# kuanyuke/BayHunter

Hardware: AMD Instinct MI355X
Metric: forward evals/sec (SWD+RF, 10-layer) (higher is better)
Workload: dtype f64; 1 GPU; joint10: rdispph+prf(201 samples, nsamp 512), 10 layers, 21 periods, 524288 models/GPU/step; models_per_gpu=524288, err_models=0, library=bayhunter_amd 0.2 (gfx950) src 067974131c026079, overlap=True

## Files before the change

### bayhunter_amd/csrc/kernels.hip

```cpp
#include <hip/hip_runtime.h>
#include <cstdlib>
#include "kernels.h"
#include "rf_core.h"
#include "swd_core.h"
#include "swd_team.h"

namespace bh {

static hipError_t ensure_dyn_lds(const void *func, size_t lds, size_t (&set)[16])
{
    if (lds <= 48 * 1024) return hipSuccess;
    int dev = 0;
    hipError_t e = hipGetDevice(&dev);
    if (e != hipSuccess) return e;
    dev &= 15;
    if (lds > set[dev]) {
        e = hipFuncSetAttribute(func, hipFuncAttributeMaxDynamicSharedMemorySize, (int)lds);
        if (e != hipSuccess) return e;
        set[dev] = lds;
    }
    return hipSuccess;
}

struct LdsLay {
    float *base;
    int L;
    __device__ __forceinline__ float d(int i) const { return base[(0 * L + i) * SWD_T]; }
    __device__ __forceinline__ float a(int i) const { return base[(1 * L + i) * SWD_T]; }
    __device__ __forceinline__ float b(int i) const { return base[(2 * L + i) * SWD_T]; }
    __device__ __forceinline__ float rho(int i) const { return base[(3 * L + i) * SWD_T]; }
    __device__ __forceinline__ void set_d(int i, float v) { base[(0 * L + i) * SWD_T] = v; }
    __device__ __forceinline__ void set_a(int i, float v) { base[(1 * L + i) * SWD_T] = v; }
    __device__ __forceinline__ void set_b(int i, float v) { base[(2 * L + i) * SWD_T] = v; }
    __device__ __forceinline__ void set_rho(int i, float v) { base[(3 * L + i) * SWD_T] = v; }
};

__device__ __forceinline__ void swd_bad_depth(const SwdArgs &A, const SwdTargetDev &tg, int t, long b)
{
    double *out = A.out + b * A.out_stride + tg.out_off;
    for (int k = 0; k < tg.nper; k++) out[k] = __builtin_nan("");
    A.err[b * A.ntargets + t] = 2;
}

struct QueueSrc {
    const SwdArgs &A;
    const SwdTargetDev &tg;
    unsigned int *counter;
    int t;
    long cur;
    __device__ __forceinline__ int next(LdsLay &lay, double *&out, double *&cws, double *&cbws)
    {
        unsigned int b;
        int nl;
        const int L = A.Lmax;
        for (;;) {
            b = atomicAdd(counter, 1u);
            if (b >= (unsigned int)A.B) return 0;
            if (A.order) b = (unsigned int)A.order[b];
            nl = A.nlay[b];
            if (nl >= 1 && nl <= L) break;
            swd_bad_depth(A, tg, t, b);
        }
        cur = b;
        const long g = (long)b * A.mstride;
        if (A.vec2) {
            constexpr int CH = 6;
            for (int l0 = 0; l0 < nl; l0 += 2 * CH) {
                double2 p[CH], q[CH];
#pragma unroll
                for (int u = 0; u < CH; u++)
                    if (l0 + 2 * u < nl) {
                        p[u] = *(const double2 *)(A.h + g + l0 + 2 * u);
                        q[u] = *(const double2 *)(A.vp + g + l0 + 2 * u);
                    }
#pragma unroll
                for (int u = 0; u < CH; u++) {
                    const int l = l0 + 2 * u;
                    if (l < nl) { lay.set_d(l, (float)p[u].x); lay.set_a(l, (float)q[u].x); }
                    if (l + 1 < nl) { lay.set_d(l + 1, (float)p[u].y); lay.set_a(l + 1, (float)q[u].y); }
                }
#pragma unroll
                for (int u = 0; u < CH; u++)
                    if (l0 + 2 * u < nl) {
                        p[u] = *(const double2 *)(A.vs + g + l0 + 2 * u);
                        q[u] = *(const double2 *)(A.rho + g + l0 + 2 * u);
                    }
#pragma unroll
                for (int u = 0; u < CH; u++) {
                    const int l = l0 + 2 * u;
                    if (l < nl) { lay.set_b(l, (float)p[u].x); lay.set_rho(l, (float)q[u].x); }
                    if (l + 1 < nl) { lay.set_b(l + 1, (float)p[u].y); lay.set_rho(l + 1, (float)q[u].y); }
                }
            }
        } else {
            for (int l = 0; l < nl; l++) {
                lay.set_d(l, (float)A.h[g + l]);
                lay.set_a(l, (float)A.vp[g + l]);
                lay.set_b(l, (float)A.vs[g + l]);
                lay.set_rho(l, (float)A.rho[g + l]);
            }
        }
        out = A.out + (long)b * A.out_stride + tg.out_off;
        if (tg.mode > 1) {
            cws = A.ws + ((long)t * 2 * BH_NP) * A.B + b;
            cbws = cws + (long)BH_NP * A.B;
        }
        return nl;
    }
    float *stage;
    __device__ __forceinline__ void put(SwdState &S, int k, int kmax, float v)
    {
        if (stage) stage[(k - 1) * SWD_T] = v;
        else swd_put_direct(S, k, kmax, v);
    }
    __device__ __forceinline__ void fill_zero(SwdState &S, int k, int kmax)
    {
        if (stage) { for (int i = k; i <= kmax; i++) stage[(i - 1) * SWD_T] = 0.f; }
        else swd_zero_direct(S, k, kmax);
    }
    __device__ __forceinline__ void done(int err)
    {
        A.err[cur * A.ntargets + t] = err;
        if (stage) {
            const int n = tg.nper;
            double *o = A.out + cur * A.out_stride + tg.out_off;
            int k = 0;
            if (((unsigned long long)o & 15) && n > 0) { o[0] = (double)stage[0]; k = 1; }
            for (; k + 1 < n; k += 2) swd_store_pair(o + k, stage[k * SWD_T], stage[(k + 1) * SWD_T]);
            if (k < n) o[k] = (double)stage[k * SWD_T];
        }
    }
    __device__ __forceinline__ void sphere(LdsLay &lay, int mmax, int ifunc) { swd_sphere(lay, mmax, ifunc); }
};

#ifndef BH_SWD_WAVES
#define BH_SWD_WAVES 2
#endif
#if defined(BH_LANE_PROFILE)
__device__ unsigned long long g_lane_prof[8];
template <class Lay, class Src>
__device__ __forceinline__ void swd_lane_prof(Lay &lay, Src &src, const SwdTargetDev &tg, const double *BH_RESTRICT per, int wss)
{
    SwdState S;
    swd_state_init(S);
    NevRegs nv;
    swd_nev_init(nv);
    nv.cycles = 0;
    unsigned long long td = 0, te = 0, tc = 0, n = 0, t0 = clock64(), t1;
    for (;;) {
        swd_events(S, lay, src, tg, per, wss);
        t1 = clock64(); td += t1 - t0; t0 = t1;
        if (S.st == SWD_ST_DONE) break;
        const double wvno = S.omega / S.ceval;
        const double del = (tg.iwave == 1) ? swd_dltar1(lay, S.mmax, S.llw, wvno, S.omega)
                                           : swd_dltar4(lay, S.mmax, S.llw, wvno, S.omega);
        t1 = clock64(); te += t1 - t0; t0 = t1;
        swd_control(S, del, nv);
        t1 = clock64(); tc += t1 - t0; t0 = t1;
        n++;
    }
    atomicAdd(&g_lane_prof[0], td);
    atomicAdd(&g_lane_prof[1], te);
    atomicAdd(&g_lane_prof[2], tc);
    atomicAdd(&g_lane_prof[3], n);
    atomicAdd(&g_lane_prof[4], nv.cycles);
}
extern "C" int bh_debug_lane_profile(unsigned long long *out, int reset)
{
    if (out && hipMemcpyFromSymbol(out, HIP_SYMBOL(g_lane_prof), sizeof(g_lane_prof)) != hipSuccess) return 1;
    if (reset) {
        unsigned long long z[8] = {0};
        if (hipMemcpyToSymbol(HIP_SYMBOL(g_lane_prof), z, sizeof(z)) != hipSuccess) return 1;
    }
    return 0;
}
#endif
__global__ __launch_bounds__(SWD_T) __attribute__((amdgpu_waves_per_eu(BH_SWD_WAVES, BH_SWD_WAVES))) void swd_kernel(SwdArgs A)
{
    extern __shared__ float lds[];
    const int t = blockIdx.y;
    if (!((A.tmask >> t) & 1u)) return;
    const SwdTargetDev tg = A.tg[t];
    LdsLay lay{lds + threadIdx.x, A.Lmax};
    QueueSrc src{A, tg, A.counters + t, t, 0, A.stage ? lds + 4 * A.Lmax * SWD_T + threadIdx.x : nullptr};
    double *perl = (double *)(lds + (4 * A.Lmax + A.stage) * SWD_T);
    for (int k = threadIdx.x; k < tg.nper; k += SWD_T) perl[k] = A.periods[tg.per_off + k];
    __syncthreads();
#if defined(BH_LANE_PROFILE)
    swd_lane_prof(lay, src, tg, perl, A.B);
#else
    swd_lane(lay, src, tg, perl, A.B, nullptr);
#endif
}

struct TeamLay {
    float *base;
    int L;
    __device__ __forceinline__ float d(int i) const { return base[i]; }
    __device__ __forceinline__ float a(int i) const { return base[L + i]; }
    __device__ __forceinline__ float b(int i) const { return base[2 * L + i]; }
    __device__ __forceinline__ float rho(int i) const { return base[3 * L + i]; }
    __device__ __forceinline__ void set_d(int i, float v) { base[i] = v; }
    __device__ __forceinline__ void set_a(int i, float v) { base[L + i] = v; }
    __device__ __forceinline__ void set_b(int i, float v) { base[2 * L + i] = v; }
    __device__ __forceinline__ void set_rho(int i, float v) { base[3 * L + i] = v; }
};

struct TeamSrc {
    const SwdArgs &A;
    const SwdTargetDev &tg;
    int t, lane, nlanes, taken;
    long b;
    unsigned int *queue;
    float *res;
    __device__ __forceinline__ int next(TeamLay &lay, double *&out, double *&cws, double *&cbws)
    {
        const int L = A.Lmax;
        int nl;
        for (;;) {
            if (queue) {
                int nb = 0;
                if (lane == 0) nb = (int)atomicAdd(queue, 1u);
                nb = __shfl(nb, (int)(threadIdx.x & 63) - lane, 64);
                if (nb >= A.B) return 0;
                b = A.order ? A.order[nb] : nb;
            } else {
                if (taken) return 0;
                taken = 1;
                if (A.order) b = A.order[b];
            }
            nl = A.nlay[b];
            if (nl >= 1 && nl <= L) break;
            if (lane == 0) swd_bad_depth(A, tg, t, b);
        }
        const long g = b * A.mstride;
        for (int l = lane; l < nl; l += nlanes) {
            lay.set_d(l, (float)A.h[g + l]);
            lay.set_a(l, (float)A.vp[g + l]);
            lay.set_b(l, (float)A.vs[g + l]);
            lay.set_rho(l, (float)A.rho[g + l]);
        }
        __syncthreads();
        out = A.out + b * A.out_stride + tg.out_off;
        if (tg.mode > 1) {
            cws = A.ws + ((long)t * 2 * BH_NP) * A.B + b;
            cbws = cws + (long)BH_NP * A.B;
        }
        return nl;
    }
    __device__ __forceinline__ void done(int err)
    {
        if (lane == 0) A.err[b * A.ntargets + t] = err;
        if (res && lane < tg.nper)
            A.out[b * A.out_stride + tg.out_off + lane] = (double)res[lane];
    }
    __device__ __forceinline__ void put(SwdState &S, int k, int kmax, float v)
    {
        if (res) { if (lane == 0) res[k - 1] = v; return; }
        if (lane == 0) swd_put_direct(S, k, kmax, v);
        else if ((k & 1) && k != kmax) S.pend = v;
    }
    __device__ __forceinline__ void fill_zero(SwdState &S, int k, int kmax)
    {
        if (res) {
            if (lane == 0)
                for (int i = k; i <= kmax; i++) res[i - 1] = 0.f;
            return;
        }
        if (lane == 0) swd_zero_direct(S, k, kmax);
    }
    __device__ __forceinline__ void sphere(TeamLay &lay, int mmax, int ifunc)
    {
        if (threadIdx.x < SWD_T) swd_sphere(lay, mmax, ifunc);
        __syncthreads();
    }
};

#if defined(BH_TEAM_PROFILE)
__device__ unsigned long long g_team_prof[20];
#define BH_TP_DECL unsigned long long tp_[18] = {0, 0, 0, 0, 0, 0, 0, 0, 0, 0, 0, 0, 0, 0, 0, 0, 0, 0}, tp_t0_ = clock64(), tp_t1_
#define BH_TP(i) (tp_t1_ = clock64(), tp_[i] += tp_t1_ - tp_t0_, tp_t0_ = tp_t1_)
#define BH_TP_COUNT(i, n) (tp_[i] += (n))
#define BH_TP_FLUSH(rounds)                                                                  \
    if (threadIdx.x == 0) {                                                                  \
        for (int i_ = 0; i_ < 18; i_++) atomicAdd(&g_team_prof[i_], tp_[i_]);                \
        atomicAdd(&g_team_prof[18], (unsigned long long)(rounds));                           \
        atomicAdd(&g_team_prof[19], 1ull);                                                   \
    }
#else
#define BH_TP_DECL
#define BH_TP(i)
#define BH_TP_COUNT(i, n)
#define BH_TP_FLUSH(rounds)
#endif

template <int TEAM>
__device__ __forceinline__ void swd_team_body(const SwdArgs &A)
{
    extern __shared__ double tlds[];
    constexpr int NSUB = SWD_T / TEAM;
    static_assert(NSUB > 1, "64 lanes and more per search: swd_teamw_body");
    const int sub = threadIdx.x / TEAM, lane = threadIdx.x % TEAM;
    const int t = blockIdx.y;
    if (!((A.tmask >> t) & 1u)) return;
    const SwdTargetDev tg = A.tg[t];
    const int nm = A.Lmax > TEAM ? A.Lmax : TEAM;
    const int per_team = nm * SWD_NCA + 2 * SWD_TEAM_NT + (4 * A.Lmax + 1) / 2;
    double *mats = tlds + (long)sub * per_team, *trials = mats + (long)nm * SWD_NCA, *dels = trials + SWD_TEAM_NT;
    TeamLay lay{(float *)(dels + SWD_TEAM_NT), A.Lmax};
    TeamSrc src{A, tg, t, lane, TEAM, 0, (long)blockIdx.x, A.counters + t, nullptr};
    const double *per = A.periods + tg.per_off;
    SwdState S;
    swd_state_init(S);
    NevRegs nv;
    swd_nev_init(nv);
    {
        bool live = true;
        for (;;) {
            if (live) {
                swd_events(S, lay, src, tg, per, A.B);
                live = S.st != SWD_ST_DONE;
            }
            if (!__any(live)) break;
            const int nt = live ? swd_team_plan(S, TEAM, trials) : 0;
            __syncthreads();
            swd_team_assemble(lay, lane, TEAM, tg.iwave, S, nt, trials, mats);
            __syncthreads();
            if (tg.iwave == 2 && 8 * nt <= TEAM) swd_team_chain_ray5(lay, lane, S, nt, trials, mats, dels);
            else swd_team_chain(lay, lane, tg.iwave, S, nt, trials, mats, dels);
            __syncthreads();
            swd_team_consume(S, nv, nt, trials, dels);
            __syncthreads();
        }
    }
}


template <int CTRL>
__device__ __forceinline__ double dpp_quad(double x)
{
    const int lo = __builtin_amdgcn_mov_dpp(__double2loint(x), CTRL, 0xF, 0xF, true);
    const int hi = __builtin_amdgcn_mov_dpp(__double2hiint(x), CTRL, 0xF, 0xF, true);
    return __hiloint2double(hi, lo);
}
__device__ __forceinline__ double readlane_d(double x, int j)
{
    const int lo = __builtin_amdgcn_readlane(__double2loint(x), j);
    const int hi = __builtin_amdgcn_readlane(__double2hiint(x), j);
    return __hiloint2double(hi, lo);
}

__device__ __forceinline__ double uni(double x)
{
    return __hiloint2double(__builtin_amdgcn_readfirstlane(__double2hiint(x)),
                            __builtin_amdgcn_readfirstlane(__double2loint(x)));
}
__device__ __forceinline__ int uni(int x) { return __builtin_amdgcn_readfirstlane(x); }
__device__ __forceinline__ float uni(float x) { return __int_as_float(__builtin_amdgcn_readfirstlane(__float_as_int(x))); }
template <class T>
__device__ __forceinline__ T *uni(T *p)
{
    const unsigned long long v = (unsigned long long)p;
    return (T *)(((unsigned long long)(unsigned)__builtin_amdgcn_readfirstlane((int)(v >> 32)) << 32) |
                 (unsigned)__builtin_amdgcn_readfirstlane((int)v));
}
struct LdsSlots {
    const double *d, *tc;
    __device__ __forceinline__ double del(int j) const { return d[j]; }
    __device__ __forceinline__ double c(int j) const { return tc[j]; }
};
struct TeamwVals {
    double mc, mom, dl;
    int nt;
    TeamwNode nd;
    unsigned long long left, right;
#if defined(BH_TEAM_PROFILE)
    unsigned long long *tp, *t0;
    __device__ __forceinline__ void probe(int i) const { const unsigned long long t = clock64(); tp[i] += t - *t0; *t0 = t; }
    __device__ __forceinline__ void count(int i, int n) const { tp[i] += n; }
#else
    __device__ __forceinline__ void probe(int) const {}
    __device__ __forceinline__ void count(int, int) const {}
#endif
    __device__ __forceinline__ int find(double om, double c) const
    {
        const unsigned long long m = __ballot(mc == c && mom == om && (int)(threadIdx.x & 63) < nt);
        return m ? __ffsll((long long)m) - 1 : -1;
    }
    __device__ __forceinline__ double del(int j) const { return readlane_d(dl, j); }
    __device__ __forceinline__ double c(int j) const { return readlane_d(mc, j); }
    __device__ __forceinline__ int go(const SwdState &, int j) const
    {
        return ((right >> j) & 1) ? SWD_GO_RIGHT : ((left >> j) & 1) ? SWD_GO_LEFT : SWD_GO_STOP;
    }
    __device__ __forceinline__ int chain_run(const SwdState &, int first, int dir, int max) const
    {
        const unsigned long long m = (dir == SWD_GO_RIGHT ? right : left) >> first;
        const unsigned long long stop = ~m & 0x5555555555555555ull;
        const int n = stop ? (__ffsll((long long)stop) - 1) >> 1 : 32;
        return n < max ? n : max;
    }
    __device__ __forceinline__ TeamwNode node(const SwdState &, int j) const
    {
        TeamwNode a;
        a.go = SWD_GO_STOP;
        a.out = __builtin_amdgcn_readlane(nd.out, j);
        a.c1 = readlane_d(nd.c1, j); a.d1 = readlane_d(nd.d1, j);
        a.c2 = readlane_d(nd.c2, j); a.d2 = readlane_d(nd.d2, j);
        a.c3n = readlane_d(nd.c3n, j);
        return a;
    }
    __device__ __forceinline__ int run(int first, int stride, int count, bool neg) const
    {
        const bool same = (mc == mc) && ((__double2hiint(dl) < 0) == neg) && (int)(threadIdx.x & 63) < nt;
        unsigned long long m = __ballot(same) >> first;
        int n;
        if (stride == 2) {
            const unsigned long long stop = ~m & 0x5555555555555555ull;
            n = stop ? (__ffsll((long long)stop) - 1) >> 1 : 32;
        } else {
            const unsigned long long stop = ~m;
            n = stop ? __ffsll((long long)stop) - 1 : 64;
        }
        return n < count ? n : count;
    }
};

template <int K>
struct SubVals {
    double mc, mom, dl;
    int nt, tl, base;
    const double *tc, *dls, *ndc;
    const int *nout;
    unsigned long long left, right;
    static constexpr unsigned long long MASK = (1ull << K) - 1;
    __device__ __forceinline__ void probe(int) const {}
    __device__ __forceinline__ void count(int, int) const {}
    __device__ __forceinline__ unsigned long long mine(bool p) const { return (__ballot(p) >> base) & MASK; }
    __device__ __forceinline__ int find(double om, double c) const
    {
        const unsigned long long m = mine(mc == c && mom == om && tl < nt);
        return m ? __ffsll((long long)m) - 1 : -1;
    }
    __device__ __forceinline__ double del(int j) const { return dls[j]; }
    __device__ __forceinline__ double c(int j) const { return tc[j]; }
    __device__ __forceinline__ int go(const SwdState &, int j) const
    {
        return ((right >> j) & 1) ? SWD_GO_RIGHT : ((left >> j) & 1) ? SWD_GO_LEFT : SWD_GO_STOP;
    }
    __device__ __forceinline__ int chain_run(const SwdState &, int first, int dir, int max) const
    {
        const unsigned long long m = (dir == SWD_GO_RIGHT ? right : left) >> first;
        const unsigned long long stop = ~m & 0x5555555555555555ull;
        const int n = stop ? (__ffsll((long long)stop) - 1) >> 1 : 32;
// ... 622 lines not shown
```

### bayhunter_amd/csrc/swd_core.h

```cpp
#pragma once
#include "bh_common.h"
#include "bh_math.h"

namespace bh {

struct VarProd {
    double a0, cpcq, cpy, cpz, cqw, cqx, xy, xz, wy, wz;
};

BH_DEV void swd_var(double p, double q, const Recip &by_ra, const Recip &by_rb, double wvno, double xka,
                    double xkb, double dpth, double *w_out, double *cosp_out, VarProd &o)
{
    const double ra = by_ra.b, rb = by_rb.b;
    double w, x, y, z, cosp, cosq, sinp, sinq, fac;
    double pex = 0.0, sex = 0.0;
    if (wvno < xka) {
        bh_sincos(p, &sinp, &cosp);
        w = qdiv(sinp, by_ra);
        x = -ra * sinp;
    } else if (wvno == xka) {
        cosp = 1.0; w = dpth; x = 0.0;
    } else {
        pex = p;
        fac = 0.0;
// ... 43 lines not shown
    const Recip by_rho = recip_of(rho);
    a.c12 = qdiv(wvno2 * v.cpy - v.cqx, by_rho);
    a.c13 = qdiv(-(twgm1 * a0pq + gammk * v.xz + wvno2 * gamm1 * v.wy), by_rho);
    a.c14 = qdiv(v.cpz - wvno2 * v.cqw, by_rho);
    a.c15 = qdiv(-(two * wvno2 * a0pq + v.xz + wvno2 * wvno2 * v.wy), recip_sq(by_rho));
    a.c21 = (gmgmk * v.cpz - gm1sq * v.cqw) * rho;
    a.c22 = v.cpcq;
    a.c23 = gammk * v.cpz - gamm1 * v.cqw;
    a.c24 = -v.wz;
    a.c41 = (gm1sq * v.cpy - gmgmk * v.cqx) * rho;
    a.c42 = -v.xy;
    a.c43 = gamm1 * v.cpy - gammk * v.cqx;
    a.c51 = -(two * gmgmk * gm1sq * a0pq + gmgmk * gmgmk * v.xz + gm1sq * gm1sq * v.wy) * rho2;
    a.c53 = -(gammk * gamm1 * twgm1 * a0pq + gam * gammk * gammk * v.xz + gamm1 * gm1sq * v.wy) * rho;
    double t = -two * wvno2;
    a.c31 = t * a.c53;
    a.c32 = t * a.c43;
    a.c33 = v.a0 + two * (v.cpcq - a.c11);
    a.c34 = t * a.c23;
    a.c35 = t * a.c13;
}

BH_DEV void swd_dunkin_apply(double e[5], const Dunkin &a)
{
    double e1 = e[0], e2 = e[1], e3 = e[2], e4 = e[3], e5 = e[4];
    double ee1 = ((((0.0 + e1 * a.c11) + e2 * a.c21) + e3 * a.c31) + e4 * a.c41) + e5 * a.c51;
    double ee2 = ((((0.0 + e1 * a.c12) + e2 * a.c22) + e3 * a.c32) + e4 * a.c42) + e5 * a.c41;
    double ee3 = ((((0.0 + e1 * a.c13) + e2 * a.c23) + e3 * a.c33) + e4 * a.c43) + e5 * a.c53;
    double ee4 = ((((0.0 + e1 * a.c14) + e2 * a.c24) + e3 * a.c34) + e4 * a.c22) + e5 * a.c21;
    double ee5 = ((((0.0 + e1 * a.c15) + e2 * a.c14) + e3 * a.c35) + e4 * a.c12) + e5 * a.c11;
    double t1 = bh_fmax(bh_fmax(bh_fmax(bh_fmax(bh_fmax(0.0, fabs(ee1)), fabs(ee2)), fabs(ee3)), fabs(ee4)), fabs(ee5));
    if (t1 < 1.e-40) t1 = 1.0;
    const Recip by_t1 = recip_of(t1);
    e[0] = qdiv(ee1, by_t1); e[1] = qdiv(ee2, by_t1); e[2] = qdiv(ee3, by_t1);
    e[3] = qdiv(ee4, by_t1); e[4] = qdiv(ee5, by_t1);
}

template <class Lay>
BH_DEV void swd_ray_layer_matrix(const Lay &lay, int i0, double wvno, double wvno2, double omega,
                                 Dunkin &a)
{
    double am = (double)lay.a(i0), bm = (double)lay.b(i0);
    double xka = xdiv(omega, am);
    double xkb = xdiv(omega, bm);
    double t = xdiv(bm, omega);
    double gammk = 2.0 * t * t;
    double gam = gammk * wvno2;
    double wvnop = wvno + xka, wvnom = fabs(wvno - xka);
    const Recip by_ra = xsqrt_recip_nz(wvnop * wvnom);
    wvnop = wvno + xkb; wvnom = fabs(wvno - xkb);
    const Recip by_rb = xsqrt_recip_nz(wvnop * wvnom);
    double dpth = (double)lay.d(i0);
    double rho1 = (double)lay.rho(i0);
    double p = by_ra.b * dpth, q = by_rb.b * dpth, w, cosp;
    VarProd v;
    swd_var(p, q, by_ra, by_rb, wvno, xka, xkb, dpth, &w, &cosp, v);
    swd_dnka(a, wvno2, gam, gammk, rho1, v);
}

template <class Lay>
BH_DEV void swd_ray_halfspace(const Lay &lay, int mmax, double wvno, double wvno2, double omega,
                              double e[5])
{
    const double am = (double)lay.a(mmax - 1), bm = (double)lay.b(mmax - 1);
    double xka = xdiv(omega, am);
    double xkb = xdiv(omega, bm);
    double wvnop = wvno + xka, wvnom = fabs(wvno - xka);
    double ra = xsqrt(wvnop * wvnom);
    wvnop = wvno + xkb; wvnom = fabs(wvno - xkb);
    double rb = xsqrt(wvnop * wvnom);
    double t = xdiv(bm, omega);
    double gammk = 2.0 * t * t, gam = gammk * wvno2, gamm1 = gam - 1.0;
    double rho1 = (double)lay.rho(mmax - 1);
    e[0] = rho1 * rho1 * (gamm1 * gamm1 - gam * gammk * ra * rb);
    e[1] = -rho1 * ra;
    e[2] = rho1 * (gamm1 - gammk * ra * rb);
    e[3] = rho1 * rb;
    e[4] = wvno2 - ra * rb;
}

template <class Lay>
BH_DEV double swd_ray_water(const Lay &lay, double wvno, double omega, const double e[5])
{
    double xka = omega / (double)lay.a(0);
    double wvnop = wvno + xka, wvnom = fabs(wvno - xka);
    double ra = sqrt(wvnop * wvnom);
    double dpth = (double)lay.d(0);
    double rho1 = (double)lay.rho(0);
    double p = ra * dpth, znul = 1.0e-05, w, cosp;
    VarProd v;
    swd_var(p, znul, recip_of(ra), recip_of(znul), wvno, xka, znul, dpth, &w, &cosp, v);
    double w0 = -rho1 * w;
    return cosp * e[0] + w0 * e[1];
}

template <class Lay>
BH_DEV double swd_dltar4(const Lay &lay, int mmax, int llw, double wvno, double omga)
{
    double e[5];
    double omega = omga;
    if (omega < 1.0e-4) omega = 1.0e-4;
    double wvno2 = wvno * wvno;
    swd_ray_halfspace(lay, mmax, wvno, wvno2, omega, e);
    for (int m = mmax - 1; m >= llw; m--) {
        Dunkin a;
        swd_ray_layer_matrix(lay, m - 1, wvno, wvno2, omega, a);
        swd_dunkin_apply(e, a);
    }
    if (llw != 1) return swd_ray_water(lay, wvno, omega, e);
    return e[0];
}

struct LoveLayer {
    double cosq, y, z, xmu;
};
template <class Lay>
BH_DEV void swd_love_layer(const Lay &lay, int i0, double wvno, double omega, LoveLayer &o)
{
    double beta1 = (double)lay.b(i0);
    double rho1 = (double)lay.rho(i0);
    double dm = (double)lay.d(i0);
    o.xmu = rho1 * beta1 * beta1;
    double xkb = xdiv(omega, beta1);
    double wvnop = wvno + xkb, wvnom = fabs(wvno - xkb);
    const Recip by_rb = xsqrt_recip_nz(wvnop * wvnom);
    const double rb = by_rb.b;
    double q = dm * rb, sinq, fac;
    if (wvno < xkb) {
        bh_sincos(q, &sinq, &o.cosq);
        o.y = qdiv(sinq, by_rb);
        o.z = -rb * sinq;
    } else if (wvno == xkb) {
        o.cosq = 1.0; o.y = dm; o.z = 0.0;
    } else {
        fac = 0.0;
        if (q < 16) fac = bh_exp_bounded(-2.0 * q);
        o.cosq = (1.0 + fac) * 0.5;
        sinq = (1.0 - fac) * 0.5;
        o.y = qdiv(sinq, by_rb);
        o.z = rb * sinq;
    }
}
BH_DEV void swd_love_apply(double &e1, double &e2, const LoveLayer &o)
{
    double e10 = e1 * o.cosq + e2 * o.xmu * o.z;
    double e20 = xdiv(e1 * o.y, o.xmu) + e2 * o.cosq;
    double xnor = fabs(e10), ynor = fabs(e20);
    if (ynor > xnor) xnor = ynor;
    if (xnor < 1.e-40) xnor = 1.0;
    const Recip by_nor = recip_of(xnor);
    e1 = qdiv(e10, by_nor);
    e2 = qdiv(e20, by_nor);
}
template <class Lay>
BH_DEV void swd_love_halfspace(const Lay &lay, int mmax, double wvno, double omega, double &e1, double &e2)
{
    double beta1 = (double)lay.b(mmax - 1), rho1 = (double)lay.rho(mmax - 1);
    double xkb = omega / beta1;
    double wvnop = wvno + xkb, wvnom = fabs(wvno - xkb);
    double rb = sqrt(wvnop * wvnom);
    e1 = rho1 * rb;
    e2 = 1.0 / (beta1 * beta1);
}

template <class Lay>
BH_DEV double swd_dltar1(const Lay &lay, int mmax, int llw, double wvno, double omega)
{
    double e1, e2;
    swd_love_halfspace(lay, mmax, wvno, omega, e1, e2);
    for (int m = mmax - 1; m >= llw; m--) {
        LoveLayer o;
        swd_love_layer(lay, m - 1, wvno, omega, o);
        swd_love_apply(e1, e2, o);
    }
    return e1;
}

BH_DEV float swd_gtsolh(float a, float b)
{
    float c = 0.95f * b;
    for (int i = 0; i < 5; i++) {
        float gamma = b / a, kappa = c / b;
        float k2 = kappa * kappa;
        float gk = gamma * kappa, gk2 = gk * gk;
        float fac1 = sqrtf(1.0f - gk2), fac2 = sqrtf(1.0f - k2);
        float tk = 2.0f - k2;
        float fr = tk * tk - 4.0f * fac1 * fac2;
        float frp = -4.0f * (2.0f - k2) * kappa + 4.0f * fac2 * gamma * gamma * kappa / fac1 +
                    4.0f * fac1 * kappa / fac2;
        frp = frp / b;
        c = c - fr / frp;
    }
    return c;
}

#if defined(BH_HOSTSIM)
BH_DEV float swd_powf(float x, float y) { return powf(x, y); }
#else
BH_DEV float swd_powf(float x, float y) { return (float)::pow((double)x, (double)y); }
#endif

template <class Lay>
#if defined(BH_HOSTSIM)
BH_DEV void swd_sphere(Lay &lay, int mmax, int ifunc)
#else
__device__ __noinline__ void swd_sphere(Lay &lay, int mmax, int ifunc)
#endif
{
    double ar = 6370.0, dr = 0.0, r0 = ar, r1, z0, z1, tmp;
    lay.set_d(mmax - 1, 1.0f);
    for (int i = 0; i < mmax; i++) {
        dr = dr + (double)lay.d(i);
        r1 = ar - dr;
        z0 = ar * log(ar / r0);
        z1 = ar * log(ar / r1);
        lay.set_d(i, (float)(z1 - z0));
        tmp = (ar + ar) / (r0 + r1);
        lay.set_a(i, (float)((double)lay.a(i) * tmp));
        lay.set_b(i, (float)((double)lay.b(i) * tmp));
        float btp = (float)tmp, rtp = lay.rho(i);
        if (ifunc == 1) {
            float x2 = btp * btp, x4 = x2 * x2, x5 = x4 * btp;
            lay.set_rho(i, rtp * (1.0f / x5));
        } else {
            lay.set_rho(i, rtp * swd_powf(btp, -2.275f));
        }
        r0 = r1;
    }
    lay.set_d(mmax - 1, 0.0f);
}

BH_DEV void swd_store_pair(double *p, float a, float b)
{
#if defined(BH_HOSTSIM)
    p[0] = (double)a; p[1] = (double)b;
#else
    typedef double d2_t __attribute__((ext_vector_type(2), aligned(8)));
    d2_t v;
    v.x = (double)a; v.y = (double)b;
    *(d2_t *)p = v;
#endif
}
BH_DEV void swd_put(double *out, int k, int kmax, float v, float &pend)
{
    if (k & 1) {
        if (k == kmax) out[k - 1] = (double)v;
        else pend = v;
    } else {
        swd_store_pair(out + k - 2, pend, v);
    }
}

struct SwdState;
BH_DEV void swd_put_direct(SwdState &S, int k, int kmax, float v);
BH_DEV void swd_zero_direct(SwdState &S, int k, int kmax);
struct SwdTargetDev {
    int iwave, igr, mode, iflsph, nper, per_off, out_off, _pad;
};

enum { SWD_MAX_BRACKET_STEPS = 100000 };
enum { SWD_ST_A = 0, SWD_ST_B = 1, SWD_ST_TOP = 2, SWD_ST_MID = 3, SWD_ST_DONE = 4 };

enum { SWD_EV_NONE = 0, SWD_EV_FETCH, SWD_EV_BEGIN_PERIOD, SWD_EV_SOLVED, SWD_EV_NOROOT };

struct SwdState {
    int mmax, llw, err;
    float betmx;
    double cc, cfail;
    double *out, *cws, *cbws;
    int iq, k, ift, pass, ifirst;
    float t1a, t1b;
    float pend;
    double omega, cprev, ck;
    int st, ev, idir, nev, nctrl, m, nbrk;
    double c1, c2, c3, del1, del2, del3, clow, del1st, ceval;
};

struct NevRegs {
    double x1, x2, x3, x4, x5, x6, x7, x8, x9, x10, x11;
    double y1, y2, y3, y4, y5, y6, y7, y8, y9, y10, y11;
#if defined(BH_LANE_PROFILE)
    unsigned long long cycles;
#endif
};
struct NevMem {
    double *x, *y;
};
BH_DEV void swd_nev_init(NevRegs &n)
{
    n.x1 = n.x2 = n.x3 = n.x4 = n.x5 = n.x6 = n.x7 = n.x8 = n.x9 = n.x10 = n.x11 = 0;
    n.y1 = n.y2 = n.y3 = n.y4 = n.y5 = n.y6 = n.y7 = n.y8 = n.y9 = n.y10 = n.y11 = 0;
}
BH_DEV void swd_nev_init(NevMem &n)
{
    for (int i = 0; i < 12; i++) { n.x[i] = 0; n.y[i] = 0; }
}

BH_DEV bool swd_neville(NevRegs &n, int &m, bool nev2, double c1, double del1, double c2, double del2,
                        double c3, double del3, double *x1)
{
#if defined(BH_LANE_PROFILE)
    const unsigned long long lp_t0 = clock64();
#endif
    double ym1;
    if (nev2) {
        ym1 = del3;
        if (m <= 3) {
            if (m == 1) { n.x2 = c3; n.y2 = del3; } else if (m == 2) { n.x3 = c3; n.y3 = del3; }
            else { n.x4 = c3; n.y4 = del3; }
        } else if (m <= 6) {
            if (m == 4) { n.x5 = c3; n.y5 = del3; } else if (m == 5) { n.x6 = c3; n.y6 = del3; }
            else { n.x7 = c3; n.y7 = del3; }
        } else {
            if (m == 7) { n.x8 = c3; n.y8 = del3; } else if (m == 8) { n.x9 = c3; n.y9 = del3; }
            else if (m == 9) { n.x10 = c3; n.y10 = del3; } else { n.x11 = c3; n.y11 = del3; }
        }
    } else {
        n.x1 = c1; n.y1 = del1; n.x2 = c2; n.y2 = del2; m = 1;
        ym1 = del2;
    }
    bool bad = false;
    const double guard = 1.0e-10 * fabs(ym1);
#define BH_NEV_STEP(J, XJ, YJ, XJ1)                                               \
    if (!bad && m >= J) {                                                         \
        double denom = ym1 - n.YJ;                                                \
        if (fabs(denom) < guard) bad = true;                                      \
        else n.XJ = (-n.YJ * n.XJ1 + ym1 * n.XJ) / denom;                         \
    }
    if (m >= 7) {
        BH_NEV_STEP(10, x10, y10, x11)
        BH_NEV_STEP(9, x9, y9, x10)
        BH_NEV_STEP(8, x8, y8, x9)
        BH_NEV_STEP(7, x7, y7, x8)
    }
    if (m >= 4) {
        BH_NEV_STEP(6, x6, y6, x7)
        BH_NEV_STEP(5, x5, y5, x6)
        BH_NEV_STEP(4, x4, y4, x5)
    }
    BH_NEV_STEP(3, x3, y3, x4)
    BH_NEV_STEP(2, x2, y2, x3)
    BH_NEV_STEP(1, x1, y1, x2)
#undef BH_NEV_STEP
    *x1 = n.x1;
#if defined(BH_LANE_PROFILE)
    {
        const unsigned long long act = __ballot(1);
        if ((int)(threadIdx.x & 63) == __ffsll((long long)act) - 1) n.cycles += clock64() - lp_t0;
    }
#endif
    return !bad;
}
BH_DEV bool swd_neville(NevMem &n, int &m, bool nev2, double c1, double del1, double c2, double del2,
                        double c3, double del3, double *x1)
{
    double ym1;
    if (nev2) {
        n.x[m + 1] = c3; n.y[m + 1] = del3;
        ym1 = del3;
    } else {
        n.x[1] = c1; n.y[1] = del1; n.x[2] = c2; n.y[2] = del2; m = 1;
        ym1 = del2;
    }
    const double guard = 1.0e-10 * fabs(ym1);
    double xj1 = n.x[m + 1];
    for (int j = m; j >= 1; j--) {
        const double yj = n.y[j];
        const double denom = ym1 - yj;
        if (fabs(denom) < guard) return false;
        xj1 = (-yj * xj1 + ym1 * n.x[j]) / denom;
        n.x[j] = xj1;
    }
    *x1 = xj1;
    return true;
}

BH_DEV void swd_nev_restart(NevMem &n, double x1, double del1, double c2, double del2)
{
    n.x[1] = x1; n.y[1] = del1; n.x[2] = c2; n.y[2] = del2;
}
BH_DEV void swd_nev_restart(NevRegs &n, double x1, double del1, double c2, double del2)
{
    n.x1 = x1; n.y1 = del1; n.x2 = c2; n.y2 = del2;
}

BH_DEV void swd_put_direct(SwdState &S, int k, int kmax, float v) { swd_put(S.out, k, kmax, v, S.pend); }
BH_DEV void swd_zero_direct(SwdState &S, int k, int kmax)
{
    if (!(k & 1)) S.out[k - 2] = (double)S.pend;
    for (int i = k; i <= kmax; i++) S.out[i - 1] = 0.0;
}

BH_DEV void swd_state_init(SwdState &S)
{
    S.mmax = 1; S.llw = 1; S.err = 0; S.betmx = 0.f; S.cc = 0; S.cfail = 0;
    S.out = nullptr; S.cws = nullptr; S.cbws = nullptr;
    S.iq = 1; S.k = 1; S.ift = 999; S.pass = 0; S.ifirst = 0; S.t1a = 0; S.t1b = 0; S.pend = 0;
    S.omega = 0; S.cprev = 0; S.ck = 0;
    S.st = SWD_ST_DONE; S.ev = SWD_EV_FETCH; S.idir = 1; S.nev = 1; S.nctrl = 1; S.m = 1; S.nbrk = 0;
    S.c1 = S.c2 = S.c3 = S.del1 = S.del2 = S.del3 = S.clow = S.del1st = S.ceval = 0;
}

BH_DEV double swd_bracket_next(double &c1, int &idir, double clow, double dc)
{
    double c2;
    for (;;) {
        c2 = (idir > 0) ? c1 + dc : c1 - dc;
        if (c2 <= clow) { idir = +1; c1 = clow; continue; }
        break;
    }
    return c2;
}

BH_DEV void swd_on_begin_period(SwdState &S, const SwdTargetDev &tg, const double *BH_RESTRICT per, int wss)
{
    const double TWOPI = 2.0 * 3.141592653589793;
    const double one = 1.0e-2;
    const double onea = 1.5;
    const double dc = (double)0.005f;
    const float h = 0.005f;
    double t1 = per[S.k - 1];
    if (tg.igr > 0) {
        S.t1a = (float)(t1 / (double)(1.f + h));
        S.t1b = (float)(t1 / (double)(1.f - h));
        t1 = (double)S.t1a;
    } else {
        S.t1a = (float)t1;
    }
    if (S.k == 1 && S.iq == 1) { S.c1 = S.cc; S.clow = S.cc; S.ifirst = 1; }
    else if (S.k == 1) { S.c1 = S.cws[0] + one * dc; S.clow = S.c1; S.ifirst = 1; }
    else if (S.iq > 1) {
        S.ifirst = 0;
        S.clow = S.cws[(S.k - 1) * wss] + one * dc;
        S.c1 = S.cprev;
        if (S.c1 < S.clow) S.c1 = S.clow;
    } else {
        S.ifirst = 0;
        S.c1 = S.cprev - onea * dc;
        S.clow = S.cc;
    }
    S.pass = 0;
    S.omega = TWOPI / t1;
    S.ceval = S.c1;
    S.st = SWD_ST_A;
    S.ev = SWD_EV_NONE;
}

template <class Src>
BH_DEV void swd_on_solved(SwdState &S, Src &src, const SwdTargetDev &tg, int wss)
{
    const double TWOPI = 2.0 * 3.141592653589793;
    const double one = 1.0e-2;
    const double onea = 1.5;
    const double dc = (double)0.005f;
    const int igr = tg.igr, kmax = tg.nper;
    const bool multimode = tg.mode > 1;
    if (S.pass == 0) {
        S.ck = S.c1;
        if (multimode) S.cws[(S.k - 1) * wss] = S.ck;
        if (igr > 0) {
            double t1 = (double)S.t1b;
            S.ifirst = 0;
            S.clow = (multimode ? S.cbws[(S.k - 1) * wss] : 0.0) + one * dc;
            S.c1 = S.c1 - onea * dc;
            S.pass = 1;
            S.omega = TWOPI / t1;
            S.ceval = S.c1;
            S.st = SWD_ST_A;
            S.ev = SWD_EV_NONE;
            return;
        }
        S.c1 = 0.0;
    } else {
        if (S.ev == SWD_EV_NOROOT) S.c1 = S.ck;
        if (multimode) S.cbws[(S.k - 1) * wss] = S.c1;
    }
    float cc0 = (float)S.ck, cc1b = (float)S.c1;
    if (igr == 0) {
        src.put(S, S.k, kmax, cc0);
    } else {
        float gvel = (1 / S.t1a - 1 / S.t1b) / (1 / (S.t1a * cc0) - 1 / (S.t1b * cc1b));
        src.put(S, S.k, kmax, gvel);
    }
    S.cprev = S.ck;
    S.k++;
    S.ev = SWD_EV_BEGIN_PERIOD;
}

template <class Lay, class Src>
BH_DEV void swd_driver(SwdState &S, Lay &lay, Src &src, const SwdTargetDev &tg,
                       const double *BH_RESTRICT per, int wss, bool allow_fetch = true)
{
    const double dc = (double)0.005f;
    const int ifunc = tg.iwave, kmax = tg.nper, nmode = tg.mode;
    const bool multimode = nmode > 1;
    while (S.ev != SWD_EV_NONE) {
        if (S.ev == SWD_EV_FETCH) {
            if (!allow_fetch) { S.st = SWD_ST_DONE; break; }
            S.mmax = src.next(lay, S.out, S.cws, S.cbws);
            if (S.mmax <= 0) { S.st = SWD_ST_DONE; S.ev = SWD_EV_NONE; break; }
            S.err = 0;
            S.llw = 1;
            if (lay.b(0) <= 0.0f) S.llw = 2;
            if (tg.iflsph == 1) src.sphere(lay, S.mmax, ifunc);
            int jmn = 0, jsol = 1;
            S.betmx = -1.e20f;
            float betmn = 1.e20f;
            for (int i = 0; i < S.mmax; i++) {
                float bi = lay.b(i), ai = lay.a(i);
                if (bi > 0.01f && bi < betmn) { betmn = bi; jmn = i; jsol = 1; }
                else if (bi <= 0.01f && ai < betmn) { betmn = ai; jmn = i; jsol = 0; }
                if (bi > S.betmx) S.betmx = bi;
            }
            float cc1 = (jsol == 0) ? betmn : swd_gtsolh(lay.a(jmn), lay.b(jmn));
            cc1 = .95f * cc1;
            cc1 = .90f * cc1;
            S.cc = (double)cc1;
            S.cfail = (double)S.betmx + dc;
            if (multimode)
                for (int i = 0; i < kmax; i++) { S.cws[i * wss] = 0.0; S.cbws[i * wss] = 0.0; }
            S.iq = 1; S.k = 1; S.ift = 999; S.c1 = S.cc;
            if (kmax > 0 && nmode > 0) S.ev = SWD_EV_BEGIN_PERIOD;
            else { src.done(S.err); S.ev = SWD_EV_FETCH; }
        } else if (S.ev == SWD_EV_BEGIN_PERIOD) {
            if (S.k > kmax) {
                S.iq++; S.k = 1;
                if (S.iq > nmode) { src.done(S.err); S.ev = SWD_EV_FETCH; }
                continue;
            }
            if (S.k >= S.ift) { S.ev = SWD_EV_NOROOT; S.pass = 0; continue; }
            swd_on_begin_period(S, tg, per, wss);
        } else if (S.ev == SWD_EV_SOLVED || (S.ev == SWD_EV_NOROOT && S.pass == 1)) {
            swd_on_solved(S, src, tg, wss);
        } else {
            if (S.iq <= 1) S.err = 1;
            S.ift = S.k;
            src.fill_zero(S, S.k, kmax);
            S.iq++; S.k = 1;
            if (S.iq > nmode) { src.done(S.err); S.ev = SWD_EV_FETCH; }
            else S.ev = SWD_EV_BEGIN_PERIOD;
        }
    }
}

template <class Lay, class Src>
BH_DEV void swd_events(SwdState &S, Lay &lay, Src &src, const SwdTargetDev &tg,
                       const double *BH_RESTRICT per, int wss, bool allow_fetch = true)
{
#if !defined(BH_NO_FAST_EVENTS)
    if (S.ev == SWD_EV_SOLVED || (S.ev == SWD_EV_NOROOT && S.pass == 1)) swd_on_solved(S, src, tg, wss);
    if (S.ev == SWD_EV_BEGIN_PERIOD && S.k <= tg.nper && S.k < S.ift) swd_on_begin_period(S, tg, per, wss);
    if (S.ev != SWD_EV_NONE)
#endif
        swd_driver(S, lay, src, tg, per, wss, allow_fetch);
}

template <class Nev>
BH_DEV void swd_control(SwdState &S, double del, Nev &nv)
{
    const double dc = (double)0.005f;
    const double pct = (double)0.01f;
    bool bracket_step = false, finish = false;
    if (S.st == SWD_ST_A) {
        S.del1 = del;
        if (S.ifirst == 1) S.del1st = S.del1;
        S.idir = (S.ifirst == 1 || !bh_signs_differ(S.del1st, S.del1)) ? +1 : -1;
        S.nbrk = 0;
        bracket_step = true;
    } else if (S.st == SWD_ST_B) {
        S.del2 = del;
        if (bh_signs_differ(S.del1, S.del2)) {
            S.c3 = 0.5 * (S.c1 + S.c2);
            S.nev = 1; S.nctrl = 1;
            S.ceval = S.c3; S.st = SWD_ST_TOP;
        } else {
            S.c1 = S.c2; S.del1 = S.del2;
            if (S.c1 < S.cc || S.c1 >= S.cfail || ++S.nbrk > SWD_MAX_BRACKET_STEPS) S.ev = SWD_EV_NOROOT;
            else bracket_step = true;
        }
    } else {
        bool mid = (S.st == SWD_ST_MID);
        S.del3 = del;
        if (!mid) {
            S.nctrl = S.nctrl + 1;
            if (S.nctrl >= 100) finish = true;
            else if (S.c3 < dmin(S.c1, S.c2) || S.c3 > dmax(S.c1, S.c2)) {
                S.nev = 0;
                S.c3 = 0.5 * (S.c1 + S.c2);
                S.ceval = S.c3; S.st = SWD_ST_MID;
            } else mid = true;
        }
        if (mid && !finish) {
            double s13 = S.del1 - S.del3, s32 = S.del3 - S.del2;
            if (bh_signs_differ(S.del3, S.del1)) { S.c2 = S.c3; S.del2 = S.del3; }
            else { S.c1 = S.c3; S.del1 = S.del3; }
            if (fabs(S.c1 - S.c2) <= 1.e-6 * S.c1) finish = true;
            else {
                if (bh_signs_differ(s13, s32)) S.nev = 0;
                double ss1 = fabs(S.del1), s1 = pct * ss1, ss2 = fabs(S.del2), s2 = pct * ss2;
                bool do_half = (s1 > ss2 || s2 > ss1 || S.nev == 0);
                if (!do_half) {
                    double x1;
                    if (swd_neville(nv, S.m, S.nev == 2, S.c1, S.del1, S.c2, S.del2, S.c3, S.del3, &x1)) {
                        S.c3 = x1;
                        S.nev = 2;
                        S.m = S.m + 1;
                        if (S.m > 10) S.m = 10;
                    } else do_half = true;
                }
                if (do_half) {
                    S.c3 = 0.5 * (S.c1 + S.c2);
                    S.nev = 1;
                    S.m = 1;
                }
                S.ceval = S.c3; S.st = SWD_ST_TOP;
            }
        }
    }
    if (bracket_step) {
        S.c2 = swd_bracket_next(S.c1, S.idir, S.clow, dc);
        S.ceval = S.c2; S.st = SWD_ST_B;
    }
    if (finish) {
        S.c1 = S.c3;
        S.ev = (S.c1 > (double)S.betmx) ? SWD_EV_NOROOT : SWD_EV_SOLVED;
    }
}

template <class Lay, class Src>
BH_DEV void swd_lane(Lay &lay, Src &src, const SwdTargetDev &tg, const double *BH_RESTRICT per,
                     int wss, long *ncalls)
{
    SwdState S;
    swd_state_init(S);
    NevRegs nv;
    swd_nev_init(nv);
    long nc = 0;
    for (;;) {
        swd_events(S, lay, src, tg, per, wss);
        if (S.st == SWD_ST_DONE) break;
        double wvno = S.omega / S.ceval;
        double del = (tg.iwave == 1) ? swd_dltar1(lay, S.mmax, S.llw, wvno, S.omega)
                                     : swd_dltar4(lay, S.mmax, S.llw, wvno, S.omega);
        nc++;
        swd_control(S, del, nv);
    }
    if (ncalls) *ncalls = nc;
}

}
```

Baseline: 9.056 million evals/s.

## Flatten SWD event driver and control into branch-free predicated passes

Replaces the while-loop event driver in the per-lane SWD root search with a single straight-line pass that runs each event handler under a predicate, looping back when events remain. It adds a predicated NevRegs overload of swd_control and rewrites the Neville update as select-based code. The aim is to cut wavefront divergence when lanes sit in different solver states. The cost is that every lane now evaluates all control paths and Neville divisions, which adds double-precision arithmetic and register pressure.

```diff
diff --git a/bayhunter_amd/csrc/kernels.hip b/bayhunter_amd/csrc/kernels.hip
--- a/bayhunter_amd/csrc/kernels.hip
+++ b/bayhunter_amd/csrc/kernels.hip
@@ -148,8 +148,9 @@
     nv.cycles = 0;
     unsigned long long td = 0, te = 0, tc = 0, n = 0, t0 = clock64(), t1;
     for (;;) {
-        swd_events(S, lay, src, tg, per, wss);
+        swd_events_pass(S, lay, src, tg, per, wss);
         t1 = clock64(); td += t1 - t0; t0 = t1;
+        if (S.ev != SWD_EV_NONE) continue;
         if (S.st == SWD_ST_DONE) break;
         const double wvno = S.omega / S.ceval;
         const double del = (tg.iwave == 1) ? swd_dltar1(lay, S.mmax, S.llw, wvno, S.omega)
diff --git a/bayhunter_amd/csrc/swd_core.h b/bayhunter_amd/csrc/swd_core.h
--- a/bayhunter_amd/csrc/swd_core.h
+++ b/bayhunter_amd/csrc/swd_core.h
@@ -369,38 +369,42 @@
 #if defined(BH_LANE_PROFILE)
     const unsigned long long lp_t0 = clock64();
 #endif
-    double ym1;
-    if (nev2) {
-        ym1 = del3;
-        if (m <= 3) {
-            if (m == 1) { n.x2 = c3; n.y2 = del3; } else if (m == 2) { n.x3 = c3; n.y3 = del3; }
-            else { n.x4 = c3; n.y4 = del3; }
-        } else if (m <= 6) {
-            if (m == 4) { n.x5 = c3; n.y5 = del3; } else if (m == 5) { n.x6 = c3; n.y6 = del3; }
-            else { n.x7 = c3; n.y7 = del3; }
-        } else {
-            if (m == 7) { n.x8 = c3; n.y8 = del3; } else if (m == 8) { n.x9 = c3; n.y9 = del3; }
-            else if (m == 9) { n.x10 = c3; n.y10 = del3; } else { n.x11 = c3; n.y11 = del3; }
+    const int mo = m;
+    const double ym1 = nev2 ? del3 : del2;
+    n.x1 = nev2 ? n.x1 : c1;
+    n.y1 = nev2 ? n.y1 : del1;
+    n.x2 = nev2 ? (mo == 1 ? c3 : n.x2) : c2;
+    n.y2 = nev2 ? (mo == 1 ? del3 : n.y2) : del2;
+    n.x3 = (nev2 & (mo == 2)) ? c3 : n.x3;
+    n.y3 = (nev2 & (mo == 2)) ? del3 : n.y3;
+    n.x4 = (nev2 & (mo == 3)) ? c3 : n.x4;
+    n.y4 = (nev2 & (mo == 3)) ? del3 : n.y4;
+    if (nev2 & (mo >= 4)) {
+#define BH_NEV_PUT(J, XJ1, YJ1) n.XJ1 = (mo == J) ? c3 : n.XJ1; n.YJ1 = (mo == J) ? del3 : n.YJ1;
+        BH_NEV_PUT(4, x5, y5) BH_NEV_PUT(5, x6, y6) BH_NEV_PUT(6, x7, y7)
+        if (mo >= 7) {
+            BH_NEV_PUT(7, x8, y8) BH_NEV_PUT(8, x9, y9) BH_NEV_PUT(9, x10, y10)
+            n.x11 = (mo >= 10) ? c3 : n.x11; n.y11 = (mo >= 10) ? del3 : n.y11;
         }
-    } else {
-        n.x1 = c1; n.y1 = del1; n.x2 = c2; n.y2 = del2; m = 1;
-        ym1 = del2;
-    }
-    bool bad = false;
+#undef BH_NEV_PUT
+    }
+    m = nev2 ? mo : 1;
+    bool live = true;
     const double guard = 1.0e-10 * fabs(ym1);
 #define BH_NEV_STEP(J, XJ, YJ, XJ1)                                               \
-    if (!bad && m >= J) {                                                         \
-        double denom = ym1 - n.YJ;                                                \
-        if (fabs(denom) < guard) bad = true;                                      \
-        else n.XJ = (-n.YJ * n.XJ1 + ym1 * n.XJ) / denom;                         \
-    }
-    if (m >= 7) {
-        BH_NEV_STEP(10, x10, y10, x11)
-        BH_NEV_STEP(9, x9, y9, x10)
-        BH_NEV_STEP(8, x8, y8, x9)
-        BH_NEV_STEP(7, x7, y7, x8)
+    {                                                                             \
+        const double denom = ym1 - n.YJ;                                          \
+        live = live & !((m >= J) & (fabs(denom) < guard));                        \
+        const double q = (-n.YJ * n.XJ1 + ym1 * n.XJ) / denom;                    \
+        n.XJ = (live & (m >= J)) ? q : n.XJ;                                      \
     }
     if (m >= 4) {
+        if (m >= 7) {
+            BH_NEV_STEP(10, x10, y10, x11)
+            BH_NEV_STEP(9, x9, y9, x10)
+            BH_NEV_STEP(8, x8, y8, x9)
+            BH_NEV_STEP(7, x7, y7, x8)
+        }
         BH_NEV_STEP(6, x6, y6, x7)
         BH_NEV_STEP(5, x5, y5, x6)
         BH_NEV_STEP(4, x4, y4, x5)
@@ -416,7 +420,7 @@
         if ((int)(threadIdx.x & 63) == __ffsll((long long)act) - 1) n.cycles += clock64() - lp_t0;
     }
 #endif
-    return !bad;
+    return live;
 }
 BH_DEV bool swd_neville(NevMem &n, int &m, bool nev2, double c1, double del1, double c2, double del2,
                         double c3, double del3, double *x1)
@@ -555,57 +559,70 @@
 }
 
 template <class Lay, class Src>
+BH_DEV void swd_on_fetch(SwdState &S, Lay &lay, Src &src, const SwdTargetDev &tg, int wss)
+{
+    const double dc = (double)0.005f;
+    const int ifunc = tg.iwave, kmax = tg.nper, nmode = tg.mode;
+    S.mmax = src.next(lay, S.out, S.cws, S.cbws);
+    if (S.mmax <= 0) { S.st = SWD_ST_DONE; S.ev = SWD_EV_NONE; return; }
+    S.err = 0;
+    S.llw = 1;
+    if (lay.b(0) <= 0.0f) S.llw = 2;
+    if (tg.iflsph == 1) src.sphere(lay, S.mmax, ifunc);
+    int jmn = 0, jsol = 1;
+    S.betmx = -1.e20f;
+    float betmn = 1.e20f;
+    for (int i = 0; i < S.mmax; i++) {
+        float bi = lay.b(i), ai = lay.a(i);
+        if (bi > 0.01f && bi < betmn) { betmn = bi; jmn = i; jsol = 1; }
+        else if (bi <= 0.01f && ai < betmn) { betmn = ai; jmn = i; jsol = 0; }
+        if (bi > S.betmx) S.betmx = bi;
+    }
+    float cc1 = (jsol == 0) ? betmn : swd_gtsolh(lay.a(jmn), lay.b(jmn));
+    cc1 = .95f * cc1;
+    cc1 = .90f * cc1;
+    S.cc = (double)cc1;
+    S.cfail = (double)S.betmx + dc;
+    if (nmode > 1)
+        for (int i = 0; i < kmax; i++) { S.cws[i * wss] = 0.0; S.cbws[i * wss] = 0.0; }
+    S.iq = 1; S.k = 1; S.ift = 999; S.c1 = S.cc;
+    if (kmax > 0 && nmode > 0) S.ev = SWD_EV_BEGIN_PERIOD;
+    else { src.done(S.err); S.ev = SWD_EV_FETCH; }
+}
+template <class Src>
+BH_DEV void swd_on_periods_done(SwdState &S, Src &src, const SwdTargetDev &tg)
+{
+    S.iq++; S.k = 1;
+    if (S.iq > tg.mode) { src.done(S.err); S.ev = SWD_EV_FETCH; }
+}
+template <class Src>
+BH_DEV void swd_on_noroot(SwdState &S, Src &src, const SwdTargetDev &tg)
+{
+    if (S.iq <= 1) S.err = 1;
+    S.ift = S.k;
+    src.fill_zero(S, S.k, tg.nper);
+    S.iq++; S.k = 1;
+    if (S.iq > tg.mode) { src.done(S.err); S.ev = SWD_EV_FETCH; }
+    else S.ev = SWD_EV_BEGIN_PERIOD;
+}
+
+template <class Lay, class Src>
 BH_DEV void swd_driver(SwdState &S, Lay &lay, Src &src, const SwdTargetDev &tg,
                        const double *BH_RESTRICT per, int wss, bool allow_fetch = true)
 {
-    const double dc = (double)0.005f;
-    const int ifunc = tg.iwave, kmax = tg.nper, nmode = tg.mode;
-    const bool multimode = nmode > 1;
+    const int kmax = tg.nper;
     while (S.ev != SWD_EV_NONE) {
         if (S.ev == SWD_EV_FETCH) {
             if (!allow_fetch) { S.st = SWD_ST_DONE; break; }
-            S.mmax = src.next(lay, S.out, S.cws, S.cbws);
-            if (S.mmax <= 0) { S.st = SWD_ST_DONE; S.ev = SWD_EV_NONE; break; }
-            S.err = 0;
-            S.llw = 1;
-            if (lay.b(0) <= 0.0f) S.llw = 2;
-            if (tg.iflsph == 1) src.sphere(lay, S.mmax, ifunc);
-            int jmn = 0, jsol = 1;
-            S.betmx = -1.e20f;
-            float betmn = 1.e20f;
-            for (int i = 0; i < S.mmax; i++) {
-                float bi = lay.b(i), ai = lay.a(i);
-                if (bi > 0.01f && bi < betmn) { betmn = bi; jmn = i; jsol = 1; }
-                else if (bi <= 0.01f && ai < betmn) { betmn = ai; jmn = i; jsol = 0; }
-                if (bi > S.betmx) S.betmx = bi;
-            }
-            float cc1 = (jsol == 0) ? betmn : swd_gtsolh(lay.a(jmn), lay.b(jmn));
-            cc1 = .95f * cc1;
-            cc1 = .90f * cc1;
-            S.cc = (double)cc1;
-            S.cfail = (double)S.betmx + dc;
-            if (multimode)
-                for (int i = 0; i < kmax; i++) { S.cws[i * wss] = 0.0; S.cbws[i * wss] = 0.0; }
-            S.iq = 1; S.k = 1; S.ift = 999; S.c1 = S.cc;
-            if (kmax > 0 && nmode > 0) S.ev = SWD_EV_BEGIN_PERIOD;
-            else { src.done(S.err); S.ev = SWD_EV_FETCH; }
+            swd_on_fetch(S, lay, src, tg, wss);
         } else if (S.ev == SWD_EV_BEGIN_PERIOD) {
-            if (S.k > kmax) {
-                S.iq++; S.k = 1;
-                if (S.iq > nmode) { src.done(S.err); S.ev = SWD_EV_FETCH; }
-                continue;
-            }
+            if (S.k > kmax) { swd_on_periods_done(S, src, tg); continue; }
             if (S.k >= S.ift) { S.ev = SWD_EV_NOROOT; S.pass = 0; continue; }
             swd_on_begin_period(S, tg, per, wss);
         } else if (S.ev == SWD_EV_SOLVED || (S.ev == SWD_EV_NOROOT && S.pass == 1)) {
             swd_on_solved(S, src, tg, wss);
         } else {
-            if (S.iq <= 1) S.err = 1;
-            S.ift = S.k;
-            src.fill_zero(S, S.k, kmax);
-            S.iq++; S.k = 1;
-            if (S.iq > nmode) { src.done(S.err); S.ev = SWD_EV_FETCH; }
-            else S.ev = SWD_EV_BEGIN_PERIOD;
+            swd_on_noroot(S, src, tg);
         }
     }
 }
@@ -620,6 +637,21 @@
     if (S.ev != SWD_EV_NONE)
 #endif
         swd_driver(S, lay, src, tg, per, wss, allow_fetch);
+}
+
+template <class Lay, class Src>
+BH_DEV void swd_events_pass(SwdState &S, Lay &lay, Src &src, const SwdTargetDev &tg,
+                            const double *BH_RESTRICT per, int wss)
+{
+    const int kmax = tg.nper;
+    if (S.ev == SWD_EV_SOLVED || (S.ev == SWD_EV_NOROOT && S.pass == 1)) swd_on_solved(S, src, tg, wss);
+    if (S.ev == SWD_EV_BEGIN_PERIOD && (S.k > kmax || S.k >= S.ift)) {
+        if (S.k > kmax) swd_on_periods_done(S, src, tg);
+        else { S.ev = SWD_EV_NOROOT; S.pass = 0; }
+    }
+    if (S.ev == SWD_EV_NOROOT && S.pass != 1) swd_on_noroot(S, src, tg);
+    if (S.ev == SWD_EV_FETCH) swd_on_fetch(S, lay, src, tg, wss);
+    if (S.ev == SWD_EV_BEGIN_PERIOD && S.k <= kmax && S.k < S.ift) swd_on_begin_period(S, tg, per, wss);
 }
 
 template <class Nev>
@@ -694,6 +726,65 @@
     }
 }
 
+BH_DEV void swd_control(SwdState &S, double del, NevRegs &nv)
+{
+    const double dc = (double)0.005f;
+    const double pct = (double)0.01f;
+    const bool isA = S.st == SWD_ST_A, isB = S.st == SWD_ST_B, isN = !(isA | isB);
+    const bool first = S.ifirst == 1;
+    const double half = 0.5 * (S.c1 + S.c2);
+    const int idirA = (first | !bh_signs_differ(S.del1st, del)) ? +1 : -1;
+    const bool brk = isB & bh_signs_differ(S.del1, del);
+    const bool scan = isB & !brk;
+    const bool outb = (S.c2 < S.cc) | (S.c2 >= S.cfail);
+    const bool noroot = scan & (outb | (S.nbrk + 1 > SWD_MAX_BRACKET_STEPS));
+    const bool bracket_step = isA | (scan & !noroot);
+    const bool top = isN & (S.st != SWD_ST_MID);
+    const int nctrl1 = S.nctrl + 1;
+    const bool fin_ctrl = top & (nctrl1 >= 100);
+    const bool tomid = top & !fin_ctrl & ((S.c3 < dmin(S.c1, S.c2)) | (S.c3 > dmax(S.c1, S.c2)));
+    const bool mid = isN & !fin_ctrl & !tomid;
+    const double s13 = S.del1 - del, s32 = del - S.del2;
+    const bool hi = bh_signs_differ(del, S.del1);
+    const double c1m = hi ? S.c1 : S.c3, del1m = hi ? S.del1 : del;
+    const double c2m = hi ? S.c3 : S.c2, del2m = hi ? del : S.del2;
+    const bool conv = fabs(c1m - c2m) <= 1.e-6 * c1m;
+    const bool refine = mid & !conv, finish = fin_ctrl | (mid & conv);
+    const int nevm = bh_signs_differ(s13, s32) ? 0 : S.nev;
+    const double ss1 = fabs(del1m), s1 = pct * ss1, ss2 = fabs(del2m), s2 = pct * ss2;
+    const bool do_half = (s1 > ss2) | (s2 > ss1) | (nevm == 0);
+    bool ok = false;
+    double x1 = 0.0;
+    int m = S.m;
+    if (refine & !do_half) ok = swd_neville(nv, m, nevm == 2, c1m, del1m, c2m, del2m, S.c3, del, &x1);
+    const double c3r = ok ? x1 : 0.5 * (c1m + c2m);
+    const bool newhalf = brk | tomid;
+    const double c3n = newhalf ? half : refine ? c3r : S.c3;
+    S.del1st = (isA & first) ? del : S.del1st;
+    S.idir = isA ? idirA : S.idir;
+    S.nbrk = isA ? 0 : (scan & !outb) ? S.nbrk + 1 : S.nbrk;
+    S.del1 = (isA | scan) ? del : mid ? del1m : S.del1;
+    S.del2 = isB ? del : mid ? del2m : S.del2;
+    S.del3 = isN ? del : S.del3;
+    S.c1 = scan ? S.c2 : mid ? c1m : S.c1;
+    S.c2 = mid ? c2m : S.c2;
+    S.c3 = c3n;
+    S.nev = brk ? 1 : tomid ? 0 : refine ? (ok ? 2 : 1) : S.nev;
+    S.m = refine ? (ok ? (m < 10 ? m + 1 : 10) : 1) : S.m;
+    S.nctrl = brk ? 1 : top ? nctrl1 : S.nctrl;
+    S.ceval = (newhalf | refine) ? c3n : S.ceval;
+    S.st = (brk | refine) ? SWD_ST_TOP : tomid ? SWD_ST_MID : S.st;
+    S.ev = noroot ? SWD_EV_NOROOT : S.ev;
+    if (bracket_step) {
+        S.c2 = swd_bracket_next(S.c1, S.idir, S.clow, dc);
+        S.ceval = S.c2; S.st = SWD_ST_B;
+    }
+    if (finish) {
+        S.c1 = S.c3;
+        S.ev = (S.c1 > (double)S.betmx) ? SWD_EV_NOROOT : SWD_EV_SOLVED;
+    }
+}
+
 template <class Lay, class Src>
 BH_DEV void swd_lane(Lay &lay, Src &src, const SwdTargetDev &tg, const double *BH_RESTRICT per,
                      int wss, long *ncalls)
@@ -704,7 +795,8 @@
     swd_nev_init(nv);
     long nc = 0;
     for (;;) {
-        swd_events(S, lay, src, tg, per, wss);
+        swd_events_pass(S, lay, src, tg, per, wss);
+        if (S.ev != SWD_EV_NONE) continue;
         if (S.st == SWD_ST_DONE) break;
         double wvno = S.omega / S.ceval;
         double del = (tg.iwave == 1) ? swd_dltar1(lay, S.mmax, S.llw, wvno, S.omega)
```

After: 9.351 million evals/s (median of 6 runs). 1.03x the previous value.
